# qpc001/Feature_Base_Pointcloud_Registration

Measured on AMD Instinct MI355X. Metric: registered scans/sec + pose RMSE vs ref, 64×1800 synthetic Velodyne, higher is better.
Workload: dtype f32; 1 GPU; C2: 64x1800 HDL-64-style scans, ~100k-pt local corner+surf map; 1024 independent scan-to-map jobs per GPU per step (C4-style independent jobs); parallelism=single GPU, imu_deskew=False, exact_voxel_order=0

## Files before the change

feature_base_pointcloud_registration_amd/api.py:

```python
import ctypes
import os

import numpy as np

from .fbr_types import (DESKEW_TABLE, IMU_SAMPLE, KEYPOSE, PF_FLOAT32, POINT_XYZI, POINT_XYZIRT, REG_STATS, FbrIcpResult,
                        FbrLoopResult, FbrParams, FbrRegStats, PointCloud2, default_params, icp_params, loop_params, ptr)

_HERE = os.path.dirname(os.path.abspath(__file__))
_LIB = None
_VP = ctypes.c_void_p
_I64 = ctypes.c_int64
_I32 = ctypes.c_int32

EXPORTED_SYMBOLS = [
    "fbr_params_default", "fbr_strerror", "fbr_abi_version", "fbr_device_count", "fbr_create",
    "fbr_destroy", "fbr_set_map", "fbr_get_map", "fbr_project", "fbr_extract_features",
    "fbr_register", "fbr_register_trace", "fbr_process_scan", "fbr_reset_stream",
    "fbr_process_batch", "fbr_ingest_bytes", "fbr_debug_counters", "fbr_map_grid_info", "fbr_batch_stage", "fbr_batch_launch", "fbr_batch_wait",
    "fbr_batch_flush", "fbr_batch_export_ready", "fbr_batch_results", "fbr_batch_set_full_masks", "fbr_batch_labels", "fbr_batch_export", "fbr_batch_bytes", "fbr_set_profiling", "fbr_set_profiling_kernels", "fbr_kernel_time", "fbr_stream",
    "fbr_voxel_grid", "fbr_affine_from_pose", "fbr_pose_from_affine", "fbr_selftest_math", "fbr_selftest_eigen6", "fbr_selftest_eig_certified", "fbr_selftest_voxel_order", "fbr_selftest_radix_sort",
    "fbr_load_map", "fbr_pcd_read", "fbr_pcd_write_ascii", "fbr_pcd_write_binary",
    "fbr_msg_to_points", "fbr_points_to_msg_data", "fbr_project_msg", "fbr_process_msg",
    "fbr_imu_convert", "fbr_imu_deskew_info", "fbr_set_deskew", "fbr_stream_copy_bandwidth", "fbr_valu_peak",
    "fbr_keyframe_params_default", "fbr_keyframes_add", "fbr_keyframes_set_pose", "fbr_keyframes_count",
    "fbr_keyframes_reset", "fbr_extract_surrounding_keyframes",
    "fbr_loop_params_default", "fbr_detect_loop_closure", "fbr_perform_loop_closure", "fbr_icp_align", "fbr_selftest_nn1",
    "fbr_comm_unique_id", "fbr_comm_create", "fbr_comm_create_local", "fbr_comm_destroy", "fbr_batch_allgather",
]


class FbrError(RuntimeError):
    def __init__(self, status, where=""):
        self.status = status
        super().__init__(f"{where}: {strerror(status)} ({status})")


def lib_path():
    return os.environ.get("FBR_LIB") or os.path.join(_HERE, "libfbr_hip.so")


def lib():
    global _LIB
    if _LIB is None:
        path = lib_path()
        if not os.path.exists(path):
            raise RuntimeError(f"{path} missing: the HIP extension is not built "
                               "(run __graft_entry__.build())")
        L = ctypes.CDLL(path)
        sig = {
            "fbr_params_default": (None, [_VP]),
            "fbr_strerror": (ctypes.c_char_p, [ctypes.c_int]),
            "fbr_abi_version": (ctypes.c_int, []),
            "fbr_device_count": (ctypes.c_int, [_VP]),
            "fbr_create": (ctypes.c_int, [_VP, _VP, ctypes.c_int]),
            "fbr_destroy": (ctypes.c_int, [_VP]),
            "fbr_set_map": (ctypes.c_int, [_VP, _VP, _I64, _VP, _I64]),
            "fbr_get_map": (ctypes.c_int, [_VP, _VP, _VP, _VP, _VP]),
            "fbr_project": (ctypes.c_int, [_VP, _VP, _I64, _VP, _VP, _VP, _VP, _VP, _VP]),
            "fbr_extract_features": (ctypes.c_int, [_VP, _VP, _VP, _VP, _VP, _VP]),
            "fbr_register": (ctypes.c_int, [_VP, _VP, _I64, _VP, _I64, _VP, _VP]),
            "fbr_register_trace": (ctypes.c_int, [_VP, _VP, _I64, _VP, _I64, _VP, _VP, _VP]),
            "fbr_process_scan": (ctypes.c_int, [_VP, _VP, _I64, ctypes.c_double, _VP, _VP]),
            "fbr_reset_stream": (ctypes.c_int, [_VP]),
            "fbr_process_batch": (ctypes.c_int, [_VP, _VP, _VP, ctypes.c_int, _VP, _VP]),
            "fbr_ingest_bytes": (ctypes.c_int, [_VP, _VP]),
            "fbr_map_grid_info": (ctypes.c_int, [_VP, _VP]),
            "fbr_debug_counters": (ctypes.c_int, [_VP, _VP, _VP, ctypes.c_int]),
            "fbr_batch_stage": (ctypes.c_int, [_VP, _VP, _VP, ctypes.c_int, _VP]),
            "fbr_batch_launch": (ctypes.c_int, [_VP]),
            "fbr_batch_wait": (ctypes.c_int, [_VP]),
            "fbr_batch_results": (ctypes.c_int, [_VP, _VP, _VP]),
            "fbr_batch_export": (ctypes.c_int, [_VP, _VP]),
            "fbr_batch_set_full_masks": (ctypes.c_int, [_VP, ctypes.c_int]),
            "fbr_batch_labels": (ctypes.c_int, [_VP, ctypes.c_int, _VP, _I64, _VP]),
            "fbr_batch_flush": (ctypes.c_int, [_VP]),
            "fbr_batch_export_ready": (ctypes.c_int, [_VP, _VP, _VP, _VP, _VP]),
            "fbr_batch_bytes": (ctypes.c_int, [_VP, _VP, _VP]),
            "fbr_set_profiling": (ctypes.c_int, [_VP, ctypes.c_int]),
            "fbr_set_profiling_kernels": (ctypes.c_int, [_VP, ctypes.c_char_p]),
            "fbr_kernel_time": (ctypes.c_int, [_VP, ctypes.c_char_p, _VP, _VP]),
            "fbr_stream": (_VP, [_VP]),
            "fbr_voxel_grid": (ctypes.c_int, [_VP, _VP, _I64, ctypes.c_float, _VP, _VP]),
            "fbr_affine_from_pose": (None, [_VP, _VP]),
            "fbr_pose_from_affine": (None, [_VP, _VP]),
            "fbr_selftest_math": (ctypes.c_int, [ctypes.c_int, _VP, _VP, _VP]),
            "fbr_selftest_eigen6": (ctypes.c_int, [ctypes.c_int, _VP, _VP]),
            "fbr_selftest_eig_certified": (ctypes.c_int, [ctypes.c_int, _VP, ctypes.c_float, _VP]),
            "fbr_selftest_voxel_order": (ctypes.c_int, [_I64, _VP, ctypes.c_int, _VP]),
            "fbr_selftest_radix_sort": (ctypes.c_int, [_I64, ctypes.c_int, ctypes.c_int, _VP, _VP]),
            "fbr_load_map": (ctypes.c_int, [_VP, ctypes.c_char_p, ctypes.c_char_p]),
            "fbr_pcd_read": (ctypes.c_int, [ctypes.c_char_p, _VP, _I64, _VP]),
            "fbr_pcd_write_ascii": (ctypes.c_int, [ctypes.c_char_p, _VP, _I64]),
            "fbr_pcd_write_binary": (ctypes.c_int, [ctypes.c_char_p, _VP, _I64]),
            "fbr_msg_to_points": (ctypes.c_int, [_VP, _VP, _I64, _VP, _VP]),
            "fbr_points_to_msg_data": (ctypes.c_int, [_VP, _I64, _VP]),
            "fbr_project_msg": (ctypes.c_int, [_VP, _VP, _VP, _VP, _VP, _VP, _VP, _VP, _VP]),
            "fbr_process_msg": (ctypes.c_int, [_VP, _VP, ctypes.c_double, _VP, _VP, _VP]),
            "fbr_imu_convert": (ctypes.c_int, [_VP, _VP, _VP]),
            "fbr_imu_deskew_info": (ctypes.c_int, [_VP, _I64, ctypes.c_double, ctypes.c_double, _VP, _VP]),
            "fbr_set_deskew": (ctypes.c_int, [_VP, _VP, ctypes.c_int]),
            "fbr_stream_copy_bandwidth": (ctypes.c_int, [ctypes.c_int, _I64, ctypes.c_int, _VP]),
            "fbr_valu_peak": (ctypes.c_int, [ctypes.c_int, ctypes.c_int, ctypes.c_int, ctypes.c_int, ctypes.c_int, _VP, _VP]),
            "fbr_keyframe_params_default": (None, [_VP]),
            "fbr_keyframes_add": (ctypes.c_int, [_VP, _VP, _VP, _I64, _VP, _I64]),
            "fbr_keyframes_set_pose": (ctypes.c_int, [_VP, _I64, _VP]),
            "fbr_keyframes_count": (ctypes.c_int, [_VP, _VP]),
            "fbr_keyframes_reset": (ctypes.c_int, [_VP]),
            "fbr_extract_surrounding_keyframes": (ctypes.c_int, [_VP, ctypes.c_double, _VP, _VP, _VP, _VP]),
            "fbr_loop_params_default": (None, [_VP]),
            "fbr_detect_loop_closure": (ctypes.c_int, [_VP, ctypes.c_double, _VP, _VP, _VP]),
            "fbr_perform_loop_closure": (ctypes.c_int, [_VP, ctypes.c_double, _VP, _VP]),
            "fbr_icp_align": (ctypes.c_int, [_VP, _VP, _I64, _VP, _I64, _VP, _VP]),
            "fbr_selftest_nn1": (ctypes.c_int, [_VP, _VP, _I64, _VP, _I64, ctypes.c_float, _VP, _VP]),
            "fbr_comm_unique_id": (ctypes.c_int, [_VP]),
            "fbr_comm_create": (ctypes.c_int, [_VP, _VP, _VP, ctypes.c_int, ctypes.c_int, ctypes.c_int]),
            "fbr_comm_create_local": (ctypes.c_int, [_VP, _VP, ctypes.c_int, ctypes.c_int]),
            "fbr_comm_destroy": (ctypes.c_int, [_VP]),
            "fbr_batch_allgather": (ctypes.c_int, [_VP, _VP, _I64, _VP, _VP, _VP]),
        }
        diag = bool(os.environ.get("FBR_LIB"))
        for name, (res, args) in sig.items():
            if diag and not hasattr(L, name):
                continue
            f = getattr(L, name)
            f.restype = res
            f.argtypes = args
        _LIB = L
    return _LIB


def strerror(status):
    return lib().fbr_strerror(status).decode()


def _check(status, where):
    if status != 0:
        raise FbrError(status, where)

# ... 3 lines not shown
    _check(lib().fbr_device_count(ctypes.byref(n)), "fbr_device_count")
    return n.value


def debug_counters(reset=False):
    v = [ctypes.c_longlong() for _ in range(3)]
    _check(lib().fbr_debug_counters(*[ctypes.byref(x) for x in v], int(reset)), "fbr_debug_counters")
    return tuple(x.value for x in v)


def host_times(reset=False):
    f = lib().fbr_diag_host_times
    f.restype, f.argtypes = ctypes.c_int, [_VP, ctypes.c_int]
    v = (ctypes.c_longlong * 4)()
    _check(f(v, int(reset)), "fbr_diag_host_times")
    return tuple(x * 1e-9 for x in v)


def wait_stats(reset=False):
    if not hasattr(lib(), "fbr_diag_wait_stats"):
        return -1, -1, -1.0, -1
    f = lib().fbr_diag_wait_stats
    f.restype, f.argtypes = ctypes.c_int, [_VP, ctypes.c_int]
    v = (ctypes.c_longlong * 4)()
    _check(f(v, int(reset)), "fbr_diag_wait_stats")
    return int(v[0]), int(v[1]), v[2] * 1e-9, int(v[3])


def batch_times(reset=False):
    f = lib().fbr_diag_batch_times
    f.restype, f.argtypes = ctypes.c_int, [_VP, ctypes.c_int]
    v = (ctypes.c_longlong * 2)()
    _check(f(v, int(reset)), "fbr_diag_batch_times")
    return tuple(x * 1e-9 for x in v)


def knn_tile_stats(reset=False):
    f = lib().fbr_diag_knn_tile_stats
    f.restype, f.argtypes = ctypes.c_int, [_VP, ctypes.c_int]
    v = (ctypes.c_ulonglong * 8)()
    if f(v, int(reset)) != 0:
        return None
    return tuple(int(x) for x in v)


def selftest_math(a, b):
    a = np.ascontiguousarray(a, np.float32)
    b = np.ascontiguousarray(b, np.float32)
    out = np.zeros((len(a), 6), np.float32)
    _check(lib().fbr_selftest_math(len(a), ptr(a), ptr(b), ptr(out)), "fbr_selftest_math")
    return out


def selftest_eigen6(mats):
    a = np.ascontiguousarray(mats, np.float32).reshape(-1, 36)
    out = np.zeros((len(a), 84), np.float32)
    _check(lib().fbr_selftest_eigen6(len(a), ptr(a), ptr(out)), "fbr_selftest_eigen6")
    n = len(a)
    return ((out[:, :6], out[:, 6:42].reshape(n, 6, 6)), (out[:, 42:48], out[:, 48:].reshape(n, 6, 6)))


def selftest_eig_certified(mats, thr=100.0):
    a = np.ascontiguousarray(mats, np.float32).reshape(-1, 36)
    out = np.zeros(len(a), np.int32)
    _check(lib().fbr_selftest_eig_certified(len(a), ptr(a), ctypes.c_float(thr), ptr(out)), "fbr_selftest_eig_certified")
    return out


def selftest_voxel_order(keys, lds=False):
    k = np.ascontiguousarray(keys, np.uint32)
    perm = np.zeros(len(k), np.uint32)
    _check(lib().fbr_selftest_voxel_order(len(k), ptr(k), int(lds), ptr(perm)), "fbr_selftest_voxel_order")
    return perm[np.argsort(k[perm], kind="stable")].astype(np.int64)


def selftest_radix_sort(keys, nbits, variant):
    k = np.ascontiguousarray(keys, np.uint32).copy()
    perm = np.zeros(len(k), np.uint32)
    _check(lib().fbr_selftest_radix_sort(len(k), int(nbits), int(variant), ptr(k), ptr(perm)), "fbr_selftest_radix_sort")
    return k, perm.astype(np.int64)


def stream_copy_bandwidth(device=0, nbytes=2 << 30, iters=20):
    g = ctypes.c_double()
    _check(lib().fbr_stream_copy_bandwidth(device, nbytes, iters, ctypes.byref(g)), "fbr_stream_copy_bandwidth")
    return g.value


def valu_peak(device=0, waves_per_simd=4, kind=0, iters=4096, reps=5):
    g, ms = ctypes.c_double(), ctypes.c_double()
    _check(lib().fbr_valu_peak(device, waves_per_simd, kind, iters, reps, ctypes.byref(g), ctypes.byref(ms)),
           "fbr_valu_peak")
    return g.value, ms.value


def affine_from_pose(pose):
    m = np.zeros(16, np.float32)
    lib().fbr_affine_from_pose(ptr(np.ascontiguousarray(pose, np.float32)), ptr(m))
    return m.reshape(4, 4)


def pose_from_affine(m):
    p = np.zeros(6, np.float32)
    lib().fbr_pose_from_affine(ptr(np.ascontiguousarray(m, np.float32).reshape(16)), ptr(p))
    return p

# ... 396 lines not shown
```

feature_base_pointcloud_registration_amd/csrc/fbr_common.h:

```cpp
#pragma once
#include <hip/hip_runtime.h>
#include <float.h>
#include <limits.h>
#include <stdint.h>

#include "../../include/fbr.h"

namespace fbr {

constexpr int kEmptyOwner = 0x7F7F7F7F;
constexpr int kCornerPerSeg = 20;
constexpr int kCornerPerRing = 20 * 6;
constexpr int kMaxSegment = 512;
constexpr int kMaxW = 4096;
constexpr float kGridCell = 1.0f;

__host__ __device__ inline float sqrt_rn(float x) { return (float)sqrt((double)x); }

constexpr unsigned long long kF64KeyMax = 0x7FEFFFFFFFFFFFFFull;
__device__ __forceinline__ unsigned long long key_min(unsigned long long a, unsigned long long b) {
  double r;
  asm("v_min_f64 %0, %1, %2" : "=v"(r) : "v"(__longlong_as_double((long long)a)), "v"(__longlong_as_double((long long)b)));
  return (unsigned long long)__double_as_longlong(r);
}
__device__ __forceinline__ unsigned long long key_max(unsigned long long a, unsigned long long b) {
  double r;
  asm("v_max_f64 %0, %1, %2" : "=v"(r) : "v"(__longlong_as_double((long long)a)), "v"(__longlong_as_double((long long)b)));
  return (unsigned long long)__double_as_longlong(r);
}

__host__ __device__ inline int x86_cvt(double v) {
  if (!(v > -2147483649.0 && v < 2147483648.0)) return (int)0x80000000;
  return (int)v;
}

struct StreamState {
  float smooth4_value;
  int32_t smooth4_ind;
  int8_t picked04[8];
};

struct GnState {
  float pose[6];
  float T[12];
  float trig[6];
  int32_t active;
  int32_t iter;
  int32_t converged;
  int32_t degenerate;
  int32_t n_sel;
  int32_t status;
  float matP[36];
  float crop_min[3], crop_max[3];
  int32_t pad[2];
};

struct GridDesc {
  float origin[3];
  float inv_cell;
  float inv_x;
  int32_t dims[3];
  int32_t n_cells;
  int64_t n_points;
  int32_t sparse;
  uint32_t hmask;
};

constexpr int kChunkX = 16;
__host__ __device__ inline bool map_point_finite(const float4& p) {
  return fabsf(p.x) <= 3.402823466e38f && fabsf(p.y) <= 3.402823466e38f && fabsf(p.z) <= 3.402823466e38f;
}
constexpr unsigned long long kChunkEmpty = ~0ull;
__host__ __device__ inline unsigned long long chunk_key(int z, int y, int xc) {
  return ((unsigned long long)(unsigned)z << 48) | ((unsigned long long)(unsigned)y << 24) | (unsigned long long)(unsigned)xc;
}
__host__ __device__ inline uint32_t chunk_hash(unsigned long long k) {
  return (uint32_t)((k * 0x9E3779B97F4A7C15ull) >> 32);
}

}
```

feature_base_pointcloud_registration_amd/csrc/k_project.hip:

```cpp
#include <algorithm>
#include <cstdlib>

#include "fbr_common.h"
#include "fbr_fdlibm.h"
#include "fbr_imu.h"
#include "fbr_kernels.h"

namespace fbr {

__device__ __forceinline__ bool project_xyzr(float x, float y, float z, int rowIdn, int H, int W, int& row, int& colo) {
  if (rowIdn < 0 || rowIdn >= H) return false;
  float horizonAngle = (float)((double)(fd_atan2f(x, y) * 180.0f) / M_PI);
  float ang_res_x = (float)(360.0 / (double)(float)W);
  int columnIdn = x86_cvt(-round(((double)horizonAngle - 90.0) / (double)ang_res_x) + (double)(W / 2));
  if (columnIdn >= W) columnIdn -= W;
  if (columnIdn < 0 || columnIdn >= W) return false;
  if (x * x + y * y + z * z < 1.0f) return false;
  row = rowIdn;
  colo = columnIdn;
  return true;
}

__device__ __forceinline__ bool project_point(const fbr_point_xyzirt& q, int H, int W, int& row, int& colo) {
  return project_xyzr(q.x, q.y, q.z, q.ring, H, W, row, colo);
}

constexpr int kProjThreads = 256, kProjPPT = 8, kProjChunk = kProjThreads * kProjPPT;

template <bool kPk>
__global__ void __launch_bounds__(kProjThreads) __attribute__((amdgpu_waves_per_eu(6, 8)))
k_project(const void* __restrict__ src, const int64_t* __restrict__ nin, int64_t nmax, int H, int W,
          int tile_log2, int32_t* __restrict__ owner, int32_t* __restrict__ err, int64_t n_single, OwnerTag ot) {
  extern __shared__ int32_t tile[];
  __shared__ int32_t cellk[kProjChunk];
  __shared__ int red[2][kProjThreads / 64];
  const int job = blockIdx.y, tid = threadIdx.x, lane = tid & 63, wv = tid >> 6;
  if (err && blockIdx.x == 0 && tid == 0) err[job] = 0;
  const int tcols = 1 << tile_log2, tcells = H << tile_log2, tpitch = tcols + 1;
  const int64_t n = n_single >= 0 ? n_single : nin[job];
  const fbr_point_xyzirt* P = static_cast<const fbr_point_xyzirt*>(src) + (int64_t)job * nmax;
  const float4* PK = static_cast<const float4*>(src) + (int64_t)job * nmax;
  int32_t* O = owner + (int64_t)job * H * W;
  for (int64_t base = (int64_t)blockIdx.x * kProjChunk; base < n; base += (int64_t)gridDim.x * kProjChunk) {
    int cmin = INT_MAX, cmax = -1;
    float px[kProjPPT], py[kProjPPT], pz[kProjPPT];
    int pr[kProjPPT];
#pragma unroll
    for (int k = 0; k < kProjPPT; ++k) {
      const int64_t i = base + k * kProjThreads + tid;
      const int64_t ic = i < n ? i : n - 1;
      if constexpr (kPk) {
        const float4 q = PK[ic];
        px[k] = q.x;
        py[k] = q.y;
        pz[k] = q.z;
        pr[k] = i < n ? __float_as_int(q.w) : -1;
      } else {
        const float2 xy = *reinterpret_cast<const float2*>(&P[ic].x);
        px[k] = xy.x;
        py[k] = xy.y;
        pz[k] = P[ic].z;
        pr[k] = i < n ? (int)P[ic].ring : -1;
      }
    }
#pragma unroll
    for (int k = 0; k < kProjPPT; ++k) {
      int row, col, v = -1;
      if (project_xyzr(px[k], py[k], pz[k], pr[k], H, W, row, col)) {
        v = (row << 16) | col;
        cmin = min(cmin, col);
        cmax = max(cmax, col);
      }
      cellk[k * kProjThreads + tid] = v;
    }
    for (int o = 32; o > 0; o >>= 1) {
      cmin = min(cmin, __shfl_xor(cmin, o));
      cmax = max(cmax, __shfl_xor(cmax, o));
    }
    if (lane == 0) {
      red[0][wv] = cmin;
      red[1][wv] = cmax;
    }
    __syncthreads();
    cmin = red[0][0];
    cmax = red[1][0];
    for (int w = 1; w < kProjThreads / 64; ++w) {
      cmin = min(cmin, red[0][w]);
      cmax = max(cmax, red[1][w]);
    }
    if (cmax >= 0 && cmax - cmin < tcols) {
      for (int e = tid; e < H * tpitch; e += kProjThreads) tile[e] = kEmptyOwner;
      __syncthreads();
      for (int k = 0; k < kProjPPT; ++k) {
        const int v = cellk[k * kProjThreads + tid];
        if (v >= 0)
          atomicMin(&tile[(v >> 16) * tpitch + ((v & 0xFFFF) - cmin)], (int32_t)(base + k * kProjThreads + tid));
      }
      __syncthreads();
      for (int e = tid; e < tcells; e += kProjThreads) {
        const int32_t v = tile[(e >> tile_log2) * tpitch + (e & (tcols - 1))];
        if (v != kEmptyOwner) atomicMin(&O[(e >> tile_log2) * W + cmin + (e & (tcols - 1))], (int32_t)(ot.bits | (uint32_t)v));
      }
    } else {
      for (int k = 0; k < kProjPPT; ++k) {
        const int v = cellk[k * kProjThreads + tid];
        if (v >= 0) atomicMin(&O[(v >> 16) * W + (v & 0xFFFF)], (int32_t)(ot.bits | (uint32_t)(base + k * kProjThreads + tid)));
      }
    }
    __syncthreads();
  }
}

struct CompactTile {
  int hb, cg;
};
inline CompactTile compact_tile(int H, int cells) {
  CompactTile t;
  t.hb = std::min(std::min(H, 64), cells / 32);
  t.cg = 32;
  while (t.cg < 256 && 2 * t.cg * t.hb <= cells) t.cg *= 2;
  return t;
}
__host__ __device__ inline int compact_nchunk(int cg, int W) { return (W + cg - 1) / cg; }

__global__ void k_rowcount(const int32_t* __restrict__ owner, int H, int W, int cg, int32_t* __restrict__ rowcnt,
                           int32_t* __restrict__ rowmin, int32_t* __restrict__ choff, OwnerTag ot) {
  const int row = blockIdx.x, job = blockIdx.y, lane = threadIdx.x;
  const int32_t* O = owner + ((int64_t)job * H + row) * W;
  const int nch = compact_nchunk(cg, W);
  int32_t* CH = choff + ((int64_t)job * H + row) * nch;
  int run = 0, mn = kEmptyOwner;
  for (int c00 = 0; c00 < W; c00 += 256) {
    int32_t o4[4];
#pragma unroll
    for (int q = 0; q < 4; ++q) {
      const int c = c00 + 64 * q + lane;
// ... 100 lines not shown
    const int base = scan[0] + scan[1] + scan[2] + scan[3];
    const int v = tid < nr ? rcv : 0;
    int inc = v;
    for (int sh = 1; sh < 64; sh <<= 1) {
      const int y = __shfl_up(inc, sh);
      if (lane >= sh) inc += y;
    }
    if (tid < nr) {
      const int roff = base + inc - v;
      rowoff[tid] = roff + cho;
      if (ch == 0) {
        start_ring[job * H + r0 + tid] = roff - 1 + 5;
        end_ring[job * H + r0 + tid] = roff + v - 1 - 5;
        if (r0 + tid == H - 1) nvalid[job] = roff + v;
      }
    }
  }
  const fbr_point_xyzirt* P = pts + (int64_t)job * nmax;
  const bool dsk = kDesk && (desk.mode[job] & kDeskPoints);
  const fbr_deskew_table* DT = dsk ? desk.table + job : nullptr;
  Rot3 Ls;
  float ts[3] = {0.0f, 0.0f, 0.0f};
  if (dsk) {
    int mn = kEmptyOwner;
    for (int r = lane; r < H; r += 64) mn = min(mn, desk.rowmin[job * H + r]);
    for (int s = 32; s > 0; s >>= 1) mn = min(mn, __shfl_xor(mn, s));
    float rx = 0.0f, ry = 0.0f, rz = 0.0f;
    if (mn != kEmptyOwner) find_rotation(*DT, DT->time_scan_cur + (double)P[mn].time, &rx, &ry, &rz);
    affine_inverse(rot_rpy(rx, ry, rz), Ls, ts);
  }
  if (kDesk) {
    for (int i = tid; i < HB * CG; i += 256) {
      const int c = i / HB, r = i % HB, k = r * PC + c;
      const int32_t o = own[k];
      if (o != kEmptyOwner) {
        const fbr_point_xyzirt q = P[o];
        pxyz[k] = dsk ? deskew_point(q, *DT, Ls, ts) : make_float4(q.x, q.y, q.z, q.intensity);
        prng[k] = sqrt_rn(q.x * q.x + q.y * q.y + q.z * q.z);
      }
    }
  } else {
    for (int i0 = tid; i0 < HB * CG; i0 += 512) {
      float4 v[2];
      int kk[2];
#pragma unroll
      for (int q = 0; q < 2; ++q) {
        const int i = i0 + 256 * q, c = i / HB, r = i % HB;
        kk[q] = r * PC + (i < HB * CG ? c : CG);
        const int32_t o = i < HB * CG ? own[kk[q]] : kEmptyOwner;
        if constexpr (kPk) {
          v[q] = pk[(int64_t)job * nmax + (o != kEmptyOwner ? o : 0)];
          v[q].w = 0.0f;
        } else {
          v[q] = *reinterpret_cast<const float4*>(&P[o != kEmptyOwner ? o : 0].x);
        }
      }
#pragma unroll
      for (int q = 0; q < 2; ++q) pxyz[kk[q]] = v[q];
    }
  }
  __syncthreads();
  float4* C = cloud + job * HW;
  int32_t* CI = col + job * HW;
  float* R = range + job * HW;
  const int rpp = 256 / CG;
  const int passes = (nr + rpp - 1) / rpp;
  for (int p = 0; p < passes; ++p) {
    const int r = p * rpp + tid / CG;
    int rank = 0;
    const int c = tid % CG;
    const int k = r * PC + c;
    const bool v = r < nr && own[k] != kEmptyOwner;
    const uint64_t m = __ballot(v);
    if (CG <= 32) {
      const int sh = lane & ~31;
      const uint64_t mm = (m >> sh) & 0xFFFFFFFFull;
      rank = __popcll(mm & ((1ull << (lane & 31)) - 1ull));
    } else {
      const int wv = tid >> 6, wrow = (tid % CG) >> 6;
      scan[wv] = __popcll(m);
      __syncthreads();
      int prev = 0;
      for (int q = 0; q < wrow; ++q) prev += scan[wv - wrow + q];
      rank = prev + __popcll(m & ((1ull << lane) - 1ull));
      __syncthreads();
    }
    if (v) {
      const int dst = rowoff[r] + rank;
      const float4 p = pxyz[k];
      C[dst] = p;
      CI[dst] = c0 + c;
      R[dst] = kDesk ? prng[k] : sqrt_rn(p.x * p.x + p.y * p.y + p.z * p.z);
    }
  }
}

template <bool kAligned>
__device__ __forceinline__ float msg_f32(const uint8_t* p, int off) {
  if (off < 0) return 0.0f;
  if (kAligned) return *reinterpret_cast<const float*>(p + off);
  uint32_t u = (uint32_t)p[off] | ((uint32_t)p[off + 1] << 8) | ((uint32_t)p[off + 2] << 16) |
               ((uint32_t)p[off + 3] << 24);
  return __uint_as_float(u);
}

template <bool kAligned>
__global__ void __launch_bounds__(256)
// ... 15 lines not shown
  q.time = msg_f32<kAligned>(p, L.off[5]);
  out[i] = q;
}

void launch_unpack_msg(hipStream_t s, const uint8_t* data, const MsgDev& L, fbr_point_xyzirt* out) {
  if (L.n <= 0) return;
  bool aligned = (L.point_step % 4 == 0) && (L.row_step % 4 == 0);
  for (int k = 0; k < 6; ++k)
    if (L.off[k] >= 0) aligned = aligned && (L.off[k] % (k == 4 ? 2 : 4) == 0);
  const dim3 grid((unsigned)((L.n + 255) / 256));
  if (aligned)
    fbr_launch(k_unpack_msg<true>, grid, dim3(256), 0, s, data, L, out);
  else
    fbr_launch(k_unpack_msg<false>, grid, dim3(256), 0, s, data, L, out);
}

template <bool kPk>
__global__ void __launch_bounds__(256)
k_expand_scans(const uint8_t* __restrict__ stage, int64_t nmax, const int64_t* __restrict__ nin,
               const int64_t* __restrict__ off, int rb, void* __restrict__ dst) {
  const int64_t i = (int64_t)blockIdx.x * 256 + threadIdx.x;
  const int64_t job = blockIdx.y;
  const int64_t n = min(nin[job], nmax);
  if (i >= n) return;
  const uint8_t* r = stage + off[job];
  const float* pl = reinterpret_cast<const float*>(r);
  const int64_t m = ingest_plane(n);
  const uint16_t ring = rb == 1 ? (uint16_t)r[12 * m + i] : reinterpret_cast<const uint16_t*>(r + 12 * m)[i];
  if constexpr (kPk) {
    static_cast<float4*>(dst)[job * nmax + i] = make_float4(pl[i], pl[m + i], pl[2 * m + i], __int_as_float((int)ring));
  } else {
    fbr_point_xyzirt q;
    q.x = pl[i];
    q.y = pl[m + i];
    q.z = pl[2 * m + i];
    q.intensity = 0.0f;
    q.ring = ring;
    q.pad_ = 0;
    q.time = 0.0f;
    static_cast<fbr_point_xyzirt*>(dst)[job * nmax + i] = q;
  }
}

void launch_expand_scans(hipStream_t s, const uint8_t* stage, int64_t nmax, int B, const int64_t* nin,
                         const int64_t* off, int rb, void* out, bool pk) {
  if (B <= 0 || nmax <= 0) return;
  const dim3 grid((unsigned)((nmax + 255) / 256), B);
  if (pk)
    fbr_launch(k_expand_scans<true>, grid, dim3(256), 0, s, stage, nmax, nin, off, rb, out);
  else
    fbr_launch(k_expand_scans<false>, grid, dim3(256), 0, s, stage, nmax, nin, off, rb, out);
}

void launch_project(hipStream_t s, const fbr_point_xyzirt* pts, const int64_t* nin, int64_t nmax, int B, int H,
                    int W, int32_t* owner, int32_t* err, int64_t n_single, const float4* pk, const OwnerTag& ot) {
  int blocks = (int)((nmax + kProjChunk - 1) / kProjChunk);
  if (blocks > 1024) blocks = 1024;
  if (blocks < 1) blocks = 1;
  int tile_log2 = 6;
  while (tile_log2 > 3 && ((int64_t)H << tile_log2) > 8192) --tile_log2;
  const size_t lds = sizeof(int32_t) * (size_t)H * ((1 << tile_log2) + 1);
  if (pk)
    fbr_launch(k_project<true>, dim3(blocks, B), dim3(kProjThreads), lds, s, (const void*)pk, nin, nmax, H, W,
               tile_log2, owner, err, n_single, ot);
  else
    fbr_launch(k_project<false>, dim3(blocks, B), dim3(kProjThreads), lds, s, (const void*)pts, nin, nmax, H, W,
               tile_log2, owner, err, n_single, ot);
}

int compact_cells() {
  static const int v = [] {
    const char* e = std::getenv("FBR_COMPACT_CELLS");
    const int c = e ? std::atoi(e) : 512;
    return c >= 2048 ? 2048 : c >= 1024 ? 1024 : 512;
  }();
  return v;
}

void launch_extract(hipStream_t s, const fbr_point_xyzirt* pts, int64_t nmax, int32_t* owner, int B, int H,
                    int W, int32_t* rowcnt, int32_t* choff, float4* cloud, int32_t* col, float* range,
                    int32_t* start_ring, int32_t* end_ring, int32_t* nvalid, const DeskArgs& desk, const float4* pk,
                    const OwnerTag& ot) {
  const CompactTile T = compact_tile(H, compact_cells());
  fbr_launch(k_rowcount, dim3(H, B), dim3(64), 0, s, owner, H, W, T.cg, rowcnt, desk.mode ? desk.rowmin : nullptr,
             choff, ot);
  const int tiles = ((H + T.hb - 1) / T.hb) * compact_nchunk(T.cg, W);
  const int groups = (B + 7) / 8;
  const dim3 grid((unsigned)(groups * 8 * tiles));
  const size_t cells = (size_t)T.hb * (T.cg + 1);
  if (desk.mode)
    fbr_launch(k_compact<true>, grid, dim3(256), (uint32_t)(cells * 24), s, pts, pk, nmax, owner, rowcnt, choff, B,
               H, W, T.hb, T.cg, cloud, col, range, start_ring, end_ring, nvalid, desk, ot);
  else if (pk)
    fbr_launch(k_compact<false, true>, grid, dim3(256), (uint32_t)(cells * 20), s, pts, pk, nmax, owner, rowcnt,
               choff, B, H, W, T.hb, T.cg, cloud, col, range, start_ring, end_ring, nvalid, desk, ot);
  else
    fbr_launch(k_compact<false>, grid, dim3(256), (uint32_t)(cells * 20), s, pts, pk, nmax, owner, rowcnt, choff, B,
               H, W, T.hb, T.cg, cloud, col, range, start_ring, end_ring, nvalid, desk, ot);
}

}
```

feature_base_pointcloud_registration_amd/csrc/k_selftest.hip:

```cpp
#include <algorithm>

#include "fbr_common.h"
#include "fbr_fdlibm.h"
#include "fbr_sincosf.h"
#include "fbr_introsort.h"
#include "fbr_solvers.h"

namespace fbr {

constexpr int kSelftestMathOut = 6;

__global__ void k_selftest_math(int n, const float* a, const float* b, float* out) {
  const int i = blockIdx.x * blockDim.x + threadIdx.x;
  if (i >= n) return;
  const float x = a[i], y = b[i];
  float* o = out + (int64_t)kSelftestMathOut * i;
  o[0] = sqrt_rn(x < 0.0f ? -x : x);
  o[1] = x / y;
  o[2] = fd_atan2f(x, y);
  o[3] = x * y + y * x - x;
  o[4] = gl_sinf(x);
  o[5] = gl_cosf(x);
}

__global__ void __launch_bounds__(64) k_selftest_eigen6(const float* a, float* out) {
  __shared__ float A[36], V[36], W[6];
  __shared__ int R[6], C[6];
  const int m = blockIdx.x, lane = threadIdx.x;
  float* o = out + (int64_t)m * 84;
  if (lane == 0) {
    float Ar[36], Wr[6], Vr[36];
    for (int k = 0; k < 36; ++k) Ar[k] = a[(int64_t)m * 36 + k];
    jacobi_eigen<6>(Ar, Wr, Vr);
    for (int k = 0; k < 6; ++k) o[k] = Wr[k];
    for (int k = 0; k < 36; ++k) o[6 + k] = Vr[k];
  }
  if (lane < 36) A[lane] = a[(int64_t)m * 36 + lane];
  __syncthreads();
  jacobi_eigen_wave<6>(A, W, V, R, C);
  if (lane < 6) o[42 + lane] = W[lane];
  if (lane < 36) o[48 + lane] = V[lane];
}

__global__ void k_selftest_eig_cert(int n, const float* a, float thr, int32_t* out) {
  const int m = blockIdx.x * blockDim.x + threadIdx.x;
  if (m < n) out[m] = eig_above_certified<6>(a + (int64_t)m * 36, thr) ? 1 : 0;
}

constexpr int kIsortLdsCap = 8192;
__global__ void __launch_bounds__(1024) k_selftest_isort(uint32_t* k, uint32_t* v, int32_t* posL, int32_t* posR,
                                                         int* fa, int* fb, int n, int lds) {
  __shared__ int sh[64];
  if (!lds) {
    is_partition_phase<1024>(k, v, posL, posR, n, fa, fb, sh);
    return;
  }
  __shared__ uint32_t lk[kIsortLdsCap];
  __shared__ uint16_t lv[kIsortLdsCap], lpl[kIsortLdsCap], lpr[kIsortLdsCap];
  __shared__ int lfa[3 * (kIsortLdsCap / 17 + 2)], lfb[3 * (kIsortLdsCap / 17 + 2)];
  for (int i = threadIdx.x; i < n; i += 1024) {
    lk[i] = k[i];
    lv[i] = (uint16_t)i;
  }
  is_partition_phase<1024>((FBR_IS_LDS uint32_t*)lk, (FBR_IS_LDS uint16_t*)lv, (FBR_IS_LDS uint16_t*)lpl,
                           (FBR_IS_LDS uint16_t*)lpr, n, (FBR_IS_LDS int*)lfa, (FBR_IS_LDS int*)lfb, sh);
  for (int i = threadIdx.x; i < n; i += 1024) {
    k[i] = lk[i];
    v[i] = lv[i];
  }
}

constexpr int kIsortLdsCap2 = 1024 * 18;
__global__ void __launch_bounds__(1024) k_selftest_isort2(uint32_t* k, uint32_t* v, int32_t* posL, int32_t* posR,
                                                          int n) {
  __shared__ int sh[64];
  __shared__ uint32_t lk[kIsortLdsCap2];
  __shared__ uint16_t lv[kIsortLdsCap2];
// ... 44 lines not shown
  const int64_t nf = n / 17 + 2;
  int rc = FBR_OK;
  if (hipMalloc(&dk, 4 * n) != hipSuccess || hipMalloc(&dv, 4 * n) != hipSuccess || hipMalloc(&pl, 4 * n) != hipSuccess ||
      hipMalloc(&pr, 4 * n) != hipSuccess || hipMalloc(&fa, 3 * sizeof(int) * nf) != hipSuccess ||
      hipMalloc(&fb, 3 * sizeof(int) * nf) != hipSuccess) {
    rc = FBR_ERR_HIP;
  } else if (hipMemcpy(dk, keys, 4 * n, hipMemcpyHostToDevice) != hipSuccess ||
             hipMemcpy(dv, iv.data(), 4 * n, hipMemcpyHostToDevice) != hipSuccess) {
    rc = FBR_ERR_HIP;
  } else {
    if (lds == 3) hipLaunchKernelGGL(fbr::k_selftest_isort3, dim3(1), dim3(512), 0, 0, dk, dv, (int)n);
    else if (lds == 2) hipLaunchKernelGGL(fbr::k_selftest_isort2, dim3(1), dim3(1024), 0, 0, dk, dv, pl, pr, (int)n);
    else hipLaunchKernelGGL(fbr::k_selftest_isort, dim3(1), dim3(1024), 0, 0, dk, dv, pl, pr, fa, fb, (int)n, lds);
    if (hipMemcpy(perm, dv, 4 * n, hipMemcpyDeviceToHost) != hipSuccess) rc = FBR_ERR_HIP;
  }
  for (void* q : {(void*)dk, (void*)dv, (void*)pl, (void*)pr, (void*)fa, (void*)fb}) (void)hipFree(q);
  return rc;
}

extern "C" int fbr_selftest_eig_certified(int n, const float* a, float thr, int32_t* out) {
  if (n <= 0 || !a || !out) return FBR_ERR_INVALID_ARG;
  float* da = nullptr;
  int32_t* dout = nullptr;
  int rc = FBR_OK;
  if (hipMalloc(&da, sizeof(float) * 36 * n) != hipSuccess || hipMalloc(&dout, sizeof(int32_t) * n) != hipSuccess) {
    rc = FBR_ERR_HIP;
  } else if (hipMemcpy(da, a, sizeof(float) * 36 * n, hipMemcpyHostToDevice) != hipSuccess) {
    rc = FBR_ERR_HIP;
  } else {
    hipLaunchKernelGGL(fbr::k_selftest_eig_cert, dim3((n + 63) / 64), dim3(64), 0, 0, n, da, thr, dout);
    if (hipMemcpy(out, dout, sizeof(int32_t) * n, hipMemcpyDeviceToHost) != hipSuccess) rc = FBR_ERR_HIP;
  }
  (void)hipFree(da);
  (void)hipFree(dout);
  return rc;
}

extern "C" int fbr_selftest_math(int n, const float* a, const float* b, float* out) {
  if (n <= 0 || !a || !b || !out) return FBR_ERR_INVALID_ARG;
  float *da = nullptr, *db = nullptr, *dout = nullptr;
  int rc = FBR_OK;
  if (hipMalloc(&da, sizeof(float) * n) != hipSuccess || hipMalloc(&db, sizeof(float) * n) != hipSuccess ||
      hipMalloc(&dout, sizeof(float) * fbr::kSelftestMathOut * n) != hipSuccess) {
    rc = FBR_ERR_HIP;
  } else if (hipMemcpy(da, a, sizeof(float) * n, hipMemcpyHostToDevice) != hipSuccess ||
             hipMemcpy(db, b, sizeof(float) * n, hipMemcpyHostToDevice) != hipSuccess) {
    rc = FBR_ERR_HIP;
  } else {
    hipLaunchKernelGGL(fbr::k_selftest_math, dim3((n + 255) / 256), dim3(256), 0, 0, n, da, db, dout);
    if (hipMemcpy(out, dout, sizeof(float) * fbr::kSelftestMathOut * n, hipMemcpyDeviceToHost) != hipSuccess) rc = FBR_ERR_HIP;
  }
  (void)hipFree(da);
  (void)hipFree(db);
  (void)hipFree(dout);
  return rc;
}

extern "C" int fbr_selftest_eigen6(int n, const float* a, float* out) {
  if (n <= 0 || !a || !out) return FBR_ERR_INVALID_ARG;
  float *da = nullptr, *dout = nullptr;
  int rc = FBR_OK;
  if (hipMalloc(&da, sizeof(float) * 36 * n) != hipSuccess || hipMalloc(&dout, sizeof(float) * 84 * n) != hipSuccess) {
    rc = FBR_ERR_HIP;
  } else if (hipMemcpy(da, a, sizeof(float) * 36 * n, hipMemcpyHostToDevice) != hipSuccess) {
    rc = FBR_ERR_HIP;
  } else {
    hipLaunchKernelGGL(fbr::k_selftest_eigen6, dim3(n), dim3(64), 0, 0, da, dout);
    if (hipMemcpy(out, dout, sizeof(float) * 84 * n, hipMemcpyDeviceToHost) != hipSuccess) rc = FBR_ERR_HIP;
  }
  (void)hipFree(da);
  (void)hipFree(dout);
  return rc;
}

namespace fbr {
__global__ void __launch_bounds__(256) k_stream_copy(const float4* __restrict__ a, float4* __restrict__ b, int64_t n) {
  for (int64_t i = (int64_t)blockIdx.x * 256 + threadIdx.x; i < n; i += (int64_t)gridDim.x * 256) b[i] = a[i];
}
template <int U>
__global__ void __launch_bounds__(256) k_stream_copy_u(const float4* __restrict__ a, float4* __restrict__ b, int64_t n) {
  const int64_t base = (int64_t)blockIdx.x * 256 * U + threadIdx.x;
  float4 v[U];
#pragma unroll
  for (int u = 0; u < U; ++u) {
    const int64_t i = base + (int64_t)u * 256;
    v[u] = i < n ? a[i] : make_float4(0, 0, 0, 0);
  }
#pragma unroll
  for (int u = 0; u < U; ++u) {
    const int64_t i = base + (int64_t)u * 256;
    if (i < n) {
      __builtin_nontemporal_store(v[u].x, &b[i].x);
      __builtin_nontemporal_store(v[u].y, &b[i].y);
      __builtin_nontemporal_store(v[u].z, &b[i].z);
      __builtin_nontemporal_store(v[u].w, &b[i].w);
    }
  }
}
}

extern "C" int fbr_stream_copy_bandwidth(int hip_device, int64_t bytes, int iters, double* gbps) {
  if (bytes < 16 || iters <= 0 || !gbps) return FBR_ERR_INVALID_ARG;
  if (hipSetDevice(hip_device) != hipSuccess) return FBR_ERR_NO_DEVICE;
  const int64_t n = bytes / 16;
  float4 *a = nullptr, *b = nullptr;
  hipEvent_t e0 = nullptr, e1 = nullptr;
// ... 146 lines not shown
```

include/fbr.h:

```cpp
#ifndef FBR_H_
#define FBR_H_

#include <stdint.h>

#ifdef __cplusplus
extern "C" {
#endif

#define FBR_ABI_VERSION 4

#define FBR_OK 0
#define FBR_ERR_INVALID_ARG (-1)
#define FBR_ERR_HIP (-2)
#define FBR_ERR_NO_MAP (-3)
#define FBR_ERR_CAPACITY (-4)
#define FBR_ERR_UNSUPPORTED (-5)
#define FBR_ERR_NO_DEVICE (-6)
#define FBR_ERR_STATE (-7)
#define FBR_ERR_MSG (-8)

#define FBR_REG_OK 0
#define FBR_REG_NOT_ENOUGH_FEATURES 1
#define FBR_REG_SKIPPED_INTERVAL 2
#define FBR_REG_FEATURE_CAPACITY 3
// ... 231 lines not shown

int fbr_register(fbr_ctx* ctx, const fbr_point_xyzi* corner, int64_t n_corner,
                 const fbr_point_xyzi* surf, int64_t n_surf, float pose_inout[6],
                 fbr_reg_stats* stats);
int fbr_register_trace(fbr_ctx* ctx, const fbr_point_xyzi* corner, int64_t n_corner,
                       const fbr_point_xyzi* surf, int64_t n_surf, float pose_inout[6],
                       fbr_reg_stats* stats, float* trace);

int fbr_process_scan(fbr_ctx* ctx, const fbr_point_xyzirt* points, int64_t n_in, double stamp,
                     float pose_inout[6], fbr_reg_stats* stats);
int fbr_reset_stream(fbr_ctx* ctx);

int fbr_process_batch(fbr_ctx* ctx, const fbr_point_xyzirt* const* scans, const int64_t* n_in,
                      int n_jobs, float* poses_inout ,
                      fbr_reg_stats* stats );
int fbr_map_grid_info(fbr_ctx* ctx, int64_t info[8]);
int fbr_ingest_bytes(fbr_ctx* ctx, double* h2d_bytes);
int fbr_debug_counters(long long* launches, long long* host_syncs, long long* flag_polls, int reset);

int fbr_batch_stage(fbr_ctx* ctx, const fbr_point_xyzirt* const* scans, const int64_t* n_in,
                    int n_jobs, const float* poses_in );
int fbr_batch_launch(fbr_ctx* ctx);
int fbr_batch_flush(fbr_ctx* ctx);
int fbr_batch_wait(fbr_ctx* ctx);
int fbr_batch_results(fbr_ctx* ctx, float* poses_out ,
                      fbr_reg_stats* stats );
int fbr_batch_set_full_masks(fbr_ctx* ctx, int on);
int fbr_batch_labels(fbr_ctx* ctx, int job, int8_t* label, int64_t cap, int64_t* n_out);
int fbr_batch_export(fbr_ctx* ctx, void* device_dst);
int fbr_batch_export_ready(fbr_ctx* ctx, void* device_dst, void* wait_stream, void** export_stream,
                           int64_t* launch_id);
#define FBR_COMM_ID_BYTES 128
typedef struct fbr_comm fbr_comm;
int fbr_comm_unique_id(uint8_t id_out[FBR_COMM_ID_BYTES]);
int fbr_comm_create(fbr_comm** out, fbr_ctx* ctx, const uint8_t id[FBR_COMM_ID_BYTES], int nranks, int rank,
                    int max_jobs_per_rank);
int fbr_comm_create_local(fbr_comm** out , fbr_ctx* const* ctxs, int n, int max_jobs_per_rank);
int fbr_comm_destroy(fbr_comm* comm);
int fbr_batch_allgather(fbr_ctx* ctx, fbr_comm* comm, int64_t launch_id, void* recv, void* wait_stream,
                        void** done_stream);

int fbr_batch_bytes(fbr_ctx* ctx, double* bytes_total, double* bytes_gn);

int fbr_set_profiling(fbr_ctx* ctx, int enable);
int fbr_set_profiling_kernels(fbr_ctx* ctx, const char* names);
int fbr_kernel_time(fbr_ctx* ctx, const char* kernel, double* total_ms, int64_t* launches);
void* fbr_stream(fbr_ctx* ctx);

int fbr_voxel_grid(fbr_ctx* ctx, const fbr_point_xyzi* in, int64_t n, float leaf,
                   fbr_point_xyzi* out, int64_t* n_out);

int fbr_selftest_math(int n, const float* a, const float* b, float* out);

int fbr_selftest_eigen6(int n, const float* a, float* out);

int fbr_selftest_eig_certified(int n, const float* a, float thr, int32_t* out);

int fbr_selftest_voxel_order(int64_t n, const uint32_t* keys, int lds, uint32_t* perm);
int fbr_selftest_radix_sort(int64_t n, int nbits, int variant, uint32_t* keys_inout, uint32_t* perm);

int fbr_stream_copy_bandwidth(int hip_device, int64_t bytes, int iters, double* gbps);
int fbr_valu_peak(int hip_device, int waves_per_simd, int kind, int iters, int reps, double* ginst_per_s,
                  double* ms_per_launch);

void fbr_affine_from_pose(const float pose[6], float m[16]);
void fbr_pose_from_affine(const float m[16], float pose[6]);

#ifdef __cplusplus
}
#endif
#endif
```

Before: 144,800 scans/s.

## Compute projection column with fast float atan polynomial plus certified exact fallback

Replaces the per-point fdlibm atan2 plus double-precision rounding in the projection kernel with an fp32 minimax atan polynomial that yields the column and its fractional part. Points whose fractional part falls within a guard band of a rounding boundary are queued in shared memory and recomputed with the exact reference path, so the output should match the original bit for bit. The gain is cheaper column math in the projection stage, paid for with extra __syncthreads and a compaction pass per chunk. An env var can disable it, and a selftest entry point compares the fast and exact columns.

```diff
diff --git a/feature_base_pointcloud_registration_amd/api.py b/feature_base_pointcloud_registration_amd/api.py
--- a/feature_base_pointcloud_registration_amd/api.py
+++ b/feature_base_pointcloud_registration_amd/api.py
@@ -18,7 +18,7 @@
     "fbr_register", "fbr_register_trace", "fbr_process_scan", "fbr_reset_stream",
     "fbr_process_batch", "fbr_ingest_bytes", "fbr_debug_counters", "fbr_map_grid_info", "fbr_batch_stage", "fbr_batch_launch", "fbr_batch_wait",
     "fbr_batch_flush", "fbr_batch_export_ready", "fbr_batch_results", "fbr_batch_set_full_masks", "fbr_batch_labels", "fbr_batch_export", "fbr_batch_bytes", "fbr_set_profiling", "fbr_set_profiling_kernels", "fbr_kernel_time", "fbr_stream",
-    "fbr_voxel_grid", "fbr_affine_from_pose", "fbr_pose_from_affine", "fbr_selftest_math", "fbr_selftest_eigen6", "fbr_selftest_eig_certified", "fbr_selftest_voxel_order", "fbr_selftest_radix_sort",
+    "fbr_voxel_grid", "fbr_affine_from_pose", "fbr_pose_from_affine", "fbr_selftest_math", "fbr_selftest_project_col", "fbr_selftest_eigen6", "fbr_selftest_eig_certified", "fbr_selftest_voxel_order", "fbr_selftest_radix_sort",
     "fbr_load_map", "fbr_pcd_read", "fbr_pcd_write_ascii", "fbr_pcd_write_binary",
     "fbr_msg_to_points", "fbr_points_to_msg_data", "fbr_project_msg", "fbr_process_msg",
     "fbr_imu_convert", "fbr_imu_deskew_info", "fbr_set_deskew", "fbr_stream_copy_bandwidth", "fbr_valu_peak",
@@ -84,6 +84,7 @@
             "fbr_affine_from_pose": (None, [_VP, _VP]),
             "fbr_pose_from_affine": (None, [_VP, _VP]),
             "fbr_selftest_math": (ctypes.c_int, [ctypes.c_int, _VP, _VP, _VP]),
+            "fbr_selftest_project_col": (ctypes.c_int, [ctypes.c_int, _VP, _VP, ctypes.c_int, _VP, _VP, _VP]),
             "fbr_selftest_eigen6": (ctypes.c_int, [ctypes.c_int, _VP, _VP]),
             "fbr_selftest_eig_certified": (ctypes.c_int, [ctypes.c_int, _VP, ctypes.c_float, _VP]),
             "fbr_selftest_voxel_order": (ctypes.c_int, [_I64, _VP, ctypes.c_int, _VP]),
@@ -193,6 +194,15 @@
     return out
 
 
+def selftest_project_col(x, y, W):
+    x = np.ascontiguousarray(x, np.float32)
+    y = np.ascontiguousarray(y, np.float32)
+    fast, cert, exact = (np.zeros(len(x), np.int32) for _ in range(3))
+    _check(lib().fbr_selftest_project_col(len(x), ptr(x), ptr(y), int(W), ptr(fast), ptr(cert), ptr(exact)),
+           "fbr_selftest_project_col")
+    return fast, cert.astype(bool), exact
+
+
 def selftest_eigen6(mats):
     a = np.ascontiguousarray(mats, np.float32).reshape(-1, 36)
     out = np.zeros((len(a), 84), np.float32)
diff --git a/feature_base_pointcloud_registration_amd/csrc/fbr_common.h b/feature_base_pointcloud_registration_amd/csrc/fbr_common.h
--- a/feature_base_pointcloud_registration_amd/csrc/fbr_common.h
+++ b/feature_base_pointcloud_registration_amd/csrc/fbr_common.h
@@ -27,11 +27,6 @@
   double r;
   asm("v_max_f64 %0, %1, %2" : "=v"(r) : "v"(__longlong_as_double((long long)a)), "v"(__longlong_as_double((long long)b)));
   return (unsigned long long)__double_as_longlong(r);
-}
-
-__host__ __device__ inline int x86_cvt(double v) {
-  if (!(v > -2147483649.0 && v < 2147483648.0)) return (int)0x80000000;
-  return (int)v;
 }
 
 struct StreamState {
diff --git a/feature_base_pointcloud_registration_amd/csrc/fbr_project_col.h b/feature_base_pointcloud_registration_amd/csrc/fbr_project_col.h
--- /dev/null
+++ b/feature_base_pointcloud_registration_amd/csrc/fbr_project_col.h
@@ -0,0 +1,100 @@
+#pragma once
+#include <hip/hip_runtime.h>
+#include <math.h>
+#include <stdint.h>
+
+#include "fbr_fdlibm.h"
+
+namespace fbr {
+
+__host__ __device__ inline int x86_cvt(double v) {
+  if (!(v > -2147483649.0 && v < 2147483648.0)) return (int)0x80000000;
+  return (int)v;
+}
+
+__host__ __device__ inline float col_ang_res_x(int W) { return (float)(360.0 / (double)(float)W); }
+
+__host__ __device__ inline double column_exact_t(float x, float y, int W) {
+  float horizonAngle = (float)((double)(fd_atan2f(x, y) * 180.0f) / M_PI);
+  float ang_res_x = col_ang_res_x(W);
+  return ((double)horizonAngle - 90.0) / (double)ang_res_x;
+}
+
+__host__ __device__ inline int column_exact(float x, float y, int W) {
+  return x86_cvt(-round(column_exact_t(x, y, W)) + (double)(W / 2));
+}
+
+__host__ __device__ inline int column_wrap(int c, int W) {
+  if (c >= W) c -= W;
+  return (c < 0 || c >= W) ? -1 : c;
+}
+
+constexpr float kColGuard = 2e-3f;
+constexpr int kColFastMaxW = 4096;
+
+struct ColFast {
+  float k;
+  float qf;
+  int qi;
+  int ok;
+};
+inline ColFast col_fast_coef(int W, bool enable = true) {
+  ColFast c;
+  const double res = (double)col_ang_res_x(W);
+  const double q = 90.0 / res;
+  c.qi = (int)floor(q + 0.5);
+  c.qf = (float)(q - (double)c.qi);
+  c.k = (float)(180.0 / (M_PI * res));
+  c.ok = enable && W >= 1 && W <= kColFastMaxW;
+  return c;
+}
+
+__host__ __device__ inline bool column_fast_parts(float x, float y, const ColFast& cf, int& n, float& u) {
+  const uint32_t hx = (uint32_t)f2bits(x), hy = (uint32_t)f2bits(y);
+  const uint32_t ix = hx & 0x7fffffffu, iy = hy & 0x7fffffffu;
+  const uint32_t imax = ix > iy ? ix : iy, imin = ix > iy ? iy : ix;
+  if (imax - 0x21800000u > 0x5d800000u - 0x21800000u) return false;
+  const float mx = bits2f((int32_t)imax), mn = bits2f((int32_t)imin);
+#if defined(__HIP_DEVICE_COMPILE__)
+  const float r = mn * __builtin_amdgcn_rcpf(mx);
+#else
+  const float r = mn * (1.0f / mx);
+#endif
+  const float s = r * r;
+  float p = 0.0024567022919654846f;
+  p = fmaf(p, s, -0.01440125796943903f);
+  p = fmaf(p, s, 0.03978103771805763f);
+  p = fmaf(p, s, -0.07234838604927063f);
+  p = fmaf(p, s, 0.10498934984207153f);
+  p = fmaf(p, s, -0.14161226153373718f);
+  p = fmaf(p, s, 0.19985906779766083f);
+  p = fmaf(p, s, -0.33332598209381104f);
+  p = fmaf(p, s, 0.9999998807907104f);
+  const float a = (r * cf.k) * p;
+  int m = ix > iy ? 1 : 0;
+  bool neg = ix > iy;
+  if (hy >> 31) {
+    m = 2 - m;
+    neg = !neg;
+  }
+  if (hx >> 31) {
+    m = -m;
+    neg = !neg;
+  }
+  m -= 1;
+  const float v = fmaf((float)m, cf.qf, neg ? -a : a) + 0.5f;
+  const float fl = floorf(v);
+  u = v - fl;
+  n = m * cf.qi + (int)fl;
+  return true;
+}
+
+__host__ __device__ inline bool column_fast(float x, float y, int W, const ColFast& cf, int& col) {
+  int n;
+  float u;
+  if (!cf.ok || !column_fast_parts(x, y, cf, n, u)) return false;
+  col = W / 2 - n;
+  return u > kColGuard && u < 1.0f - kColGuard;
+}
+
+}
diff --git a/feature_base_pointcloud_registration_amd/csrc/k_project.hip b/feature_base_pointcloud_registration_amd/csrc/k_project.hip
--- a/feature_base_pointcloud_registration_amd/csrc/k_project.hip
+++ b/feature_base_pointcloud_registration_amd/csrc/k_project.hip
@@ -5,24 +5,13 @@
 #include "fbr_fdlibm.h"
 #include "fbr_imu.h"
 #include "fbr_kernels.h"
+#include "fbr_project_col.h"
 
 namespace fbr {
 
-__device__ __forceinline__ bool project_xyzr(float x, float y, float z, int rowIdn, int H, int W, int& row, int& colo) {
+__device__ __forceinline__ bool project_keep(float x, float y, float z, int rowIdn, int H) {
   if (rowIdn < 0 || rowIdn >= H) return false;
-  float horizonAngle = (float)((double)(fd_atan2f(x, y) * 180.0f) / M_PI);
-  float ang_res_x = (float)(360.0 / (double)(float)W);
-  int columnIdn = x86_cvt(-round(((double)horizonAngle - 90.0) / (double)ang_res_x) + (double)(W / 2));
-  if (columnIdn >= W) columnIdn -= W;
-  if (columnIdn < 0 || columnIdn >= W) return false;
-  if (x * x + y * y + z * z < 1.0f) return false;
-  row = rowIdn;
-  colo = columnIdn;
-  return true;
-}
-
-__device__ __forceinline__ bool project_point(const fbr_point_xyzirt& q, int H, int W, int& row, int& colo) {
-  return project_xyzr(q.x, q.y, q.z, q.ring, H, W, row, colo);
+  return !(x * x + y * y + z * z < 1.0f);
 }
 
 constexpr int kProjThreads = 256, kProjPPT = 8, kProjChunk = kProjThreads * kProjPPT;
@@ -30,11 +19,16 @@
 template <bool kPk>
 __global__ void __launch_bounds__(kProjThreads) __attribute__((amdgpu_waves_per_eu(6, 8)))
 k_project(const void* __restrict__ src, const int64_t* __restrict__ nin, int64_t nmax, int H, int W,
-          int tile_log2, int32_t* __restrict__ owner, int32_t* __restrict__ err, int64_t n_single, OwnerTag ot) {
+          int tile_log2, int32_t* __restrict__ owner, int32_t* __restrict__ err, int64_t n_single, OwnerTag ot,
+          ColFast cf) {
   extern __shared__ int32_t tile[];
   __shared__ int32_t cellk[kProjChunk];
   __shared__ int red[2][kProjThreads / 64];
+  __shared__ uint16_t plist[kProjThreads];
+  __shared__ int pcnt;
   const int job = blockIdx.y, tid = threadIdx.x, lane = tid & 63, wv = tid >> 6;
+  if (tid == 0) pcnt = 0;
+  __syncthreads();
   if (err && blockIdx.x == 0 && tid == 0) err[job] = 0;
   const int tcols = 1 << tile_log2, tcells = H << tile_log2, tpitch = tcols + 1;
   const int64_t n = n_single >= 0 ? n_single : nin[job];
@@ -63,15 +57,61 @@
         pr[k] = i < n ? (int)P[ic].ring : -1;
       }
     }
+    uint32_t pend = 0;
 #pragma unroll
     for (int k = 0; k < kProjPPT; ++k) {
-      int row, col, v = -1;
-      if (project_xyzr(px[k], py[k], pz[k], pr[k], H, W, row, col)) {
-        v = (row << 16) | col;
-        cmin = min(cmin, col);
-        cmax = max(cmax, col);
+      int v = -1;
+      if (project_keep(px[k], py[k], pz[k], pr[k], H)) {
+        int col;
+        if (column_fast(px[k], py[k], W, cf, col)) {
+          col = column_wrap(col, W);
+          if (col >= 0) {
+            v = (pr[k] << 16) | col;
+            cmin = min(cmin, col);
+            cmax = max(cmax, col);
+          }
+        } else {
+          v = -2 - pr[k];
+          pend |= 1u << k;
+        }
       }
       cellk[k * kProjThreads + tid] = v;
+    }
+    int poff = 0;
+    if (pend) poff = atomicAdd(&pcnt, __popc(pend));
+    __syncthreads();
+    const int npend = pcnt;
+    for (int r0 = 0; r0 < npend; r0 += kProjThreads) {
+      int rank = poff - r0;
+#pragma unroll
+      for (int k = 0; k < kProjPPT; ++k)
+        if (pend >> k & 1) {
+          if (rank >= 0 && rank < kProjThreads) plist[rank] = (uint16_t)(k * kProjThreads + tid);
+          ++rank;
+        }
+      __syncthreads();
+      if (r0 + tid < npend) {
+        const int slot = plist[tid];
+        const int64_t i = base + slot;
+        float x, y;
+        if constexpr (kPk) {
+          const float2 xy = *reinterpret_cast<const float2*>(&PK[i]);
+          x = xy.x;
+          y = xy.y;
+        } else {
+          const float2 xy = *reinterpret_cast<const float2*>(&P[i].x);
+          x = xy.x;
+          y = xy.y;
+        }
+        const int row = -2 - cellk[slot];
+        const int col = column_wrap(column_exact(x, y, W), W);
+        cellk[slot] = col >= 0 ? (row << 16) | col : -1;
+        if (col >= 0) {
+          cmin = min(cmin, col);
+          cmax = max(cmax, col);
+        }
+      }
+      __syncthreads();
     }
     for (int o = 32; o > 0; o >>= 1) {
       cmin = min(cmin, __shfl_xor(cmin, o));
@@ -82,6 +122,7 @@
       red[1][wv] = cmax;
     }
     __syncthreads();
+    if (tid == 0) pcnt = 0;
     cmin = red[0][0];
     cmax = red[1][0];
     for (int w = 1; w < kProjThreads / 64; ++w) {
@@ -288,7 +329,9 @@
           v[q] = pk[(int64_t)job * nmax + (o != kEmptyOwner ? o : 0)];
           v[q].w = 0.0f;
         } else {
-          v[q] = *reinterpret_cast<const float4*>(&P[o != kEmptyOwner ? o : 0].x);
+          const fbr_point_xyzirt* g = &P[o != kEmptyOwner ? o : 0];
+          const float2 xy = *reinterpret_cast<const float2*>(&g->x);
+          v[q] = make_float4(xy.x, xy.y, g->z, g->intensity);
         }
       }
 #pragma unroll
@@ -410,6 +453,14 @@
     fbr_launch(k_expand_scans<false>, grid, dim3(256), 0, s, stage, nmax, nin, off, rb, out);
 }
 
+static bool proj_fast() {
+  static const bool v = [] {
+    const char* e = std::getenv("FBR_PROJ_FAST");
+    return !(e && std::atoi(e) == 0);
+  }();
+  return v;
+}
+
 void launch_project(hipStream_t s, const fbr_point_xyzirt* pts, const int64_t* nin, int64_t nmax, int B, int H,
                     int W, int32_t* owner, int32_t* err, int64_t n_single, const float4* pk, const OwnerTag& ot) {
   int blocks = (int)((nmax + kProjChunk - 1) / kProjChunk);
@@ -418,12 +469,13 @@
   int tile_log2 = 6;
   while (tile_log2 > 3 && ((int64_t)H << tile_log2) > 8192) --tile_log2;
   const size_t lds = sizeof(int32_t) * (size_t)H * ((1 << tile_log2) + 1);
+  const ColFast cf = col_fast_coef(W, proj_fast());
   if (pk)
     fbr_launch(k_project<true>, dim3(blocks, B), dim3(kProjThreads), lds, s, (const void*)pk, nin, nmax, H, W,
-               tile_log2, owner, err, n_single, ot);
+               tile_log2, owner, err, n_single, ot, cf);
   else
     fbr_launch(k_project<false>, dim3(blocks, B), dim3(kProjThreads), lds, s, (const void*)pts, nin, nmax, H, W,
-               tile_log2, owner, err, n_single, ot);
+               tile_log2, owner, err, n_single, ot, cf);
 }
 
 int compact_cells() {
diff --git a/feature_base_pointcloud_registration_amd/csrc/k_selftest.hip b/feature_base_pointcloud_registration_amd/csrc/k_selftest.hip
--- a/feature_base_pointcloud_registration_amd/csrc/k_selftest.hip
+++ b/feature_base_pointcloud_registration_amd/csrc/k_selftest.hip
@@ -2,6 +2,7 @@
 
 #include "fbr_common.h"
 #include "fbr_fdlibm.h"
+#include "fbr_project_col.h"
 #include "fbr_sincosf.h"
 #include "fbr_introsort.h"
 #include "fbr_solvers.h"
@@ -23,6 +24,16 @@
   o[5] = gl_cosf(x);
 }
 
+__global__ void k_selftest_project_col(int n, const float* x, const float* y, int W, ColFast cf, int32_t* fast,
+                                       int32_t* cert, int32_t* exact) {
+  const int i = blockIdx.x * blockDim.x + threadIdx.x;
+  if (i >= n) return;
+  int c = INT_MIN;
+  cert[i] = column_fast(x[i], y[i], W, cf, c) ? 1 : 0;
+  fast[i] = column_wrap(c, W);
+  exact[i] = column_wrap(column_exact(x[i], y[i], W), W);
+}
+
 __global__ void __launch_bounds__(64) k_selftest_eigen6(const float* a, float* out) {
   __shared__ float A[36], V[36], W[6];
   __shared__ int R[6], C[6];
@@ -173,6 +184,32 @@
   }
   (void)hipFree(da);
   (void)hipFree(db);
+  (void)hipFree(dout);
+  return rc;
+}
+
+extern "C" int fbr_selftest_project_col(int n, const float* x, const float* y, int W, int32_t* fast_col,
+                                        int32_t* certified, int32_t* exact_col) {
+  if (n <= 0 || W <= 0 || !x || !y || !fast_col || !certified || !exact_col) return FBR_ERR_INVALID_ARG;
+  float *dx = nullptr, *dy = nullptr;
+  int32_t* dout = nullptr;
+  int rc = FBR_OK;
+  if (hipMalloc(&dx, sizeof(float) * n) != hipSuccess || hipMalloc(&dy, sizeof(float) * n) != hipSuccess ||
+      hipMalloc(&dout, sizeof(int32_t) * 3 * (size_t)n) != hipSuccess) {
+    rc = FBR_ERR_HIP;
+  } else if (hipMemcpy(dx, x, sizeof(float) * n, hipMemcpyHostToDevice) != hipSuccess ||
+             hipMemcpy(dy, y, sizeof(float) * n, hipMemcpyHostToDevice) != hipSuccess) {
+    rc = FBR_ERR_HIP;
+  } else {
+    hipLaunchKernelGGL(fbr::k_selftest_project_col, dim3((n + 255) / 256), dim3(256), 0, 0, n, dx, dy, W,
+                       fbr::col_fast_coef(W), dout, dout + n, dout + 2 * (size_t)n);
+    if (hipMemcpy(fast_col, dout, sizeof(int32_t) * n, hipMemcpyDeviceToHost) != hipSuccess ||
+        hipMemcpy(certified, dout + n, sizeof(int32_t) * n, hipMemcpyDeviceToHost) != hipSuccess ||
+        hipMemcpy(exact_col, dout + 2 * (size_t)n, sizeof(int32_t) * n, hipMemcpyDeviceToHost) != hipSuccess)
+      rc = FBR_ERR_HIP;
+  }
+  (void)hipFree(dx);
+  (void)hipFree(dy);
   (void)hipFree(dout);
   return rc;
 }
diff --git a/include/fbr.h b/include/fbr.h
--- a/include/fbr.h
+++ b/include/fbr.h
@@ -307,6 +307,9 @@
 
 int fbr_selftest_math(int n, const float* a, const float* b, float* out);
 
+int fbr_selftest_project_col(int n, const float* x, const float* y, int W, int32_t* fast_col,
+                             int32_t* certified, int32_t* exact_col);
+
 int fbr_selftest_eigen6(int n, const float* a, float* out);
 
 int fbr_selftest_eig_certified(int n, const float* a, float thr, int32_t* out);
```

Result: no change. 146,000 scans/s (median of 6 runs) (+0.8%).
